# Ryannasr11/m2-tts

Hardware: AMD Instinct MI355X
Metric: audio samples/sec (22.05 kHz) + RTF, stage1_poc batch=32 @1/2/4/8 MI355X (higher is better)
Workload: dtype f32 (split 3xf16 MFMA, fp32 accumulate); 1 GPU; stage1_poc SimpleVocoder B=32 per GPU (configs[1]); stage=s1, per_gpu_batch=32, mel_frames=500, audio_samples_per_utt=32000, parallelism=weak-scaled replicas x1 (dp1, no collective in the data path)

## Files before the change

### m2-tts_amd/csrc/m2_common.h

```cpp
#pragma once

#include <hip/hip_runtime.h>
#include <stdint.h>
#include <string>

#include "../../include/m2tts_hip.h"

namespace m2 {

constexpr int kWave = 64;
constexpr float kLnEps = 1e-5f;
constexpr float kLeaky = 0.1f;
constexpr float kMaskFill = -1e9f;

enum Act : int { ACT_NONE = 0, ACT_LEAKY = 1, ACT_TANH = 2, ACT_RELU = 3, ACT_SOFTPLUS = 4 };

void set_error(const std::string& msg);

struct Switches {
    int dur_rb = 0;
    int dur_count = -1;
    int speculative = 1;
    bool tf_chain = true;
    bool tf_layer = true;
// ... 2 lines not shown
    int tfl_rb = 0;
    int tfl_first_rb = 0;
    int tfl_rb_masked = 0;
    int tfl_rb_unmasked = 0;
    int tfl_qs2 = -1;
    int att_qt = 0;
    bool att_f32 = false;
    bool voc_perlayer = false;
    bool voc_f32 = false;
    bool voc_tail_x3 = false;
    bool voc_mid_x3 = false;
    int voc_plan = -1;
    int f32_mt = 2;
    bool f32_pair = true;
    int x3_head_prio = 0;
    bool f32_comp = true;
    int midp_nch = 0;
    int tailp_nch = 0;
    bool tailp_seven = false;
    int tailp2_nch = 0;
    bool tailp2_seven = false;
    bool head_inconv = false;
    bool headmid = true;
    int s2_mid_alt = -1;
    int s2_head_tf = 0;
    int redo_grid = -1;
    bool redo_launch = false;
    bool dur_split = true;
    bool dur_pers = true;
};
const Switches& sw();
void reload_switches();

int32_t fail(int32_t code, const char* what);
int32_t hip_status(hipError_t e, const char* where);

#define M2_CHECK_ARG(cond, msg)                      \
    do {                                             \
        if (!(cond)) return ::m2::fail(M2_E_ARG, msg); \
    } while (0)
#define M2_CHECK_SHAPE(cond, msg)                      \
    do {                                               \
        if (!(cond)) return ::m2::fail(M2_E_SHAPE, msg); \
    } while (0)
#define M2_HIP(expr)                                                   \
    do {                                                               \
// ... 5 lines not shown
        hipError_t _e = hipGetLastError();                             \
        if (_e != hipSuccess) return ::m2::hip_status(_e, name);       \
    } while (0)

__device__ __forceinline__ float apply_act(float v, int act) {
    if (act == ACT_LEAKY) return v > 0.f ? v : v * kLeaky;
    if (act == ACT_TANH) return tanhf(v);
    if (act == ACT_RELU) return v > 0.f ? v : 0.f;
    if (act == ACT_SOFTPLUS) return v > 20.f ? v : log1pf(expf(v));
    return v;
}

template <int ACT>
__device__ __forceinline__ float act_t(float v) {
    if constexpr (ACT == ACT_LEAKY) return fmaxf(v, v * kLeaky);
    else if constexpr (ACT == ACT_TANH) return tanhf(v);
    else if constexpr (ACT == ACT_RELU) return v > 0.f ? v : 0.f;
    else return v;
}

__device__ __forceinline__ int dev_frames(const int32_t* p, int cap) {
    const int t = max(1, *p);
    return t <= cap ? t : 0;
}

inline int cdiv(int a, int b) { return (a + b - 1) / b; }
inline size_t align_up(size_t v, size_t a) { return (v + a - 1) / a * a; }

struct Carve {
    char* base;
    size_t cap;
    size_t off = 0;
    bool ok = true;
    Carve(void* p, size_t n) : base(static_cast<char*>(p)), cap(n) {}
    template <typename T>
    T* take(size_t count) {
        size_t o = align_up(off, 256);
        size_t n = count * sizeof(T);
        if (o + n > cap || base == nullptr) { ok = false; off = o + n; return nullptr; }
        off = o + n;
        return reinterpret_cast<T*>(base + o);
    }
};

struct Sizer {
    size_t off = 0;
// ... 43 lines not shown
```

### m2-tts_amd/csrc/m2_runtime.hip

```cpp
#include <immintrin.h>

#include <atomic>
#include <climits>
#include <cmath>
#include <cstdlib>
#include <cstring>
#include <mutex>
#include <new>
#include <string>
#include <vector>

#include "m2_common.h"
#include "m2_model.h"
#include "transformer_fused.h"
#include "transformer_layer.h"
#include "vocoder_fused.h"

namespace m2 {

namespace {
std::atomic<const Switches*> g_swp{nullptr};
std::mutex g_sw_mu;
int env_int(const char* name, int dflt) {
    const char* e = std::getenv(name);
// ... 32 lines not shown
        const int v = std::atoi(e);
        s.tfl_qs2 = (v == 2 || v == 3 || v == 4 || v == 12) ? v : 0;
    }
    s.att_qt = env_int("M2_ATT_QT", 0);
    if (const char* e = std::getenv("M2_ATT_F32")) s.att_f32 = *e && *e != '0';
    s.voc_perlayer = env_set("M2_VOCODER_PERLAYER");
    s.voc_f32 = env_set("M2_VOC_F32");
    s.voc_tail_x3 = env_set("M2_VOC_TAIL_X3");
    s.voc_mid_x3 = env_set("M2_VOC_MID_X3");
    s.voc_plan = env_int("M2_VOC_PLAN", -1);
    s.f32_mt = env_int("M2_F32_MT", 2);
    s.f32_pair = env_int("M2_F32_PAIR", 1) != 0;
    s.f32_comp = env_int("M2_F32_COMP", 1) != 0;
    s.x3_head_prio = env_int("M2_X3_HEAD_PRIO", 0);
    const int mn = env_int("M2_MIDP_NCH", 0);
    s.midp_nch = mn > 0 ? mn : 0;
    const int tn = env_int("M2_TAILP_NCH", 0);
    s.tailp_nch = tn > 0 ? tn : 0;
    s.tailp_seven = env_set("M2_TAILP_SEVEN");
    s.tailp2_nch = env_int("M2_TAILP2_NCH", 0);
    s.tailp2_seven = env_set("M2_TAILP2_SEVEN");
    s.head_inconv = env_set("M2_HEAD_INCONV");
    if (const char* e = std::getenv("M2_HEADMID"); e && (e[0] == '0' || e[0] == '1') && !e[1]) s.headmid = e[0] == '1';
    const int malt = env_int("M2_S2_MID_ALT", -1);
    s.s2_mid_alt = (malt == 0 || malt == 1) ? malt : -1;
    const int htf = env_int("M2_S2_HEAD_TF", env_set("M2_S2_HEAD_TF16") ? 16 : 0);
    s.s2_head_tf = (htf == 16 || htf == 19 || htf == 24 || htf == 27) ? htf : 0;
    s.redo_grid = env_int("M2_REDO_GRID", -1);
    s.redo_launch = env_set("M2_REDO_LAUNCH");
    s.dur_split = env_on("M2_DUR_SPLIT", true);
    s.dur_pers = env_on("M2_DUR_PERS", true);
    std::lock_guard<std::mutex> lk(g_sw_mu);
    const Switches* cur = g_swp.load(std::memory_order_relaxed);
    if (cur && std::memcmp(cur, &s, sizeof(Switches)) == 0) {
        std::free(raw);
        return;
    }
    g_swp.store(&s, std::memory_order_release);
}

int32_t launch_embed_pe(const int64_t*, const float*, const float*, int, int, int, int, float*, const int64_t*,
                        uint8_t*, hipStream_t);
int32_t launch_layer_norm(const float*, const float*, const float*, int, int, float*, hipStream_t);
int32_t launch_linear(const float*, const float*, const float*, const float*, const float*,
                      const float*, int, int, int, int, float*, hipStream_t);
int32_t launch_attention(const float*, const uint8_t*, int, int, int, int, float*, hipStream_t, bool force_f32 = false);
// ... 1259 lines not shown
```

### m2-tts_amd/csrc/vocoder_midp.h

```cpp
#pragma once
#include "m2_common.h"
#include "vocoder_fused.h"
#include "vocoder_pipe.h"

namespace m2 {
namespace mp {

using namespace pipe;

constexpr int RROWS = 64;
constexpr int RS0 = 288;
constexpr int RS1 = 544;

struct RingLay {
    static constexpr bool PLANES = false;
    static constexpr int R0_OFF = 0, R1_OFF = RROWS * RS0, R2_OFF = R1_OFF + RROWS * RS1;
    static constexpr int U_OFF = 0;
    static constexpr int LDS_BYTES = R2_OFF + RROWS * RS1;
};

constexpr int PROWS = 64, PRS = 288;

__device__ __forceinline__ unsigned r12_at(int row, int u) { return row * RS1 + 16 * (u ^ ((row >> 2) & 1)); }

template <int L, int S, class Lay = RingLay, int HB = 0, int NH = 2>
__device__ __forceinline__ void layer_role(unsigned char* lds, int qa, int L1, int nch, bool edge,
                                           const u32x4* __restrict__ W, const float* __restrict__ bias,
                                           unsigned char* __restrict__ u2row, int xown) {
    constexpr int NKB = mkb(L);
    constexpr bool PL = L == 0 && Lay::PLANES;
    constexpr int IN_OFF = L == 0 ? Lay::R0_OFF : (L == 1 ? Lay::R1_OFF : Lay::R2_OFF);
    constexpr int LO_IN = L == 0 ? 128 : 256;
    const int lane = threadIdx.x & 63, li = lane & 15, g = lane >> 4;
    u32x4 a[NH][NKB][2];
    float bv[NH][4];
#pragma unroll
    for (int hh = 0; hh < NH; ++hh) {
        const int h = HB + hh;
#pragma unroll
        for (int kb = 0; kb < NKB; ++kb) {
            const int u = munit0(L) + (2 * S + h) * NKB + kb;
            a[hh][kb][0] = W[u * 128 + lane];
            a[hh][kb][1] = W[u * 128 + 64 + lane];
        }
#pragma unroll
        for (int r = 0; r < 4; ++r) bv[hh][r] = bias[L * 128 + 32 * S + 16 * h + 4 * g + r];
    }
    unsigned radr[NKB][4], xadr[4], oadr[4];
#pragma unroll
    for (int j = 0; j < 4; ++j) {
#pragma unroll
        for (int kb = 0; kb < NKB; ++kb) {
            const MSlot sl = mslot(L, S, kb, g);
            if constexpr (PL) {
                const int e0 = li + sl.dq + 3, v = e0 & 3, row0 = (e0 >> 2) + (v >= 2 ? 1 : 0);
                radr[kb][j] = Lay::U_OFF + (v * PROWS + row0) * PRS + 16 * (sl.oct ^ (((row0 >> 2) + j) & 1));
            } else {
                const int row = (16 * j + li + sl.dq - 1) & (RROWS - 1);
                radr[kb][j] = IN_OFF + (L == 0 ? row * RS0 + sl.oct * 16 : r12_at(row, sl.oct));
            }
        }
        xadr[j] = Lay::R1_OFF + r12_at((16 * j + li - 2) & (RROWS - 1), 4 * S + g);
        oadr[j] = (L == 0 ? Lay::R1_OFF : Lay::R2_OFF) +
                  r12_at((16 * j + li) & (RROWS - 1), 4 * S + 16 * (g & 1) + (g >> 1));
    }
    u32x4 aid[NH];
// ... 43 lines not shown
#pragma unroll
            for (int r = 0; r < 4; ++r) v[r] = acc[hh][r];
            if constexpr (L < 2) {
                leaky4(v);
                if (straddle) {
                    const int x = x0 + li;
                    if (x < 0 || x >= L1) {
#pragma unroll
                        for (int r = 0; r < 4; ++r) v[r] = 0.f;
                    }
                }
            }
            unsigned h0, h1, l0, l1;
            split2u(v[0], v[1], h0, l0);
            split2u(v[2], v[3], h1, l1);
            const auto s0 = __builtin_amdgcn_permlane16_swap(h0, l0, false, false);
            const auto s1 = __builtin_amdgcn_permlane16_swap(h1, l1, false, false);
            const u32x4 val{s0[0], s1[0], s0[1], s1[1]};
            if constexpr (L < 2) {
                *reinterpret_cast<u32x4*>(lds + oadr[j] + 32 * h) = val;
            } else {
                const int x = x0 + li;
                if (k >= 0 && x >= 0 && x < xown)
                    *reinterpret_cast<u32x4*>(u2row + ((size_t)4 * x + S) * 128 + 32 * h + 64 * (g & 1) +
                                              16 * (g >> 1)) = val;
            }
        }
    };
    const int LAST = nch + 2;
    auto step = [&](int s, auto jc) {
        if (s <= LAST) {
            const int k = s - (L + 1);
            if (k >= -1 && k < nch) work(k, jc);
            step_barrier();
        }
    };
    constexpr int J0 = (-1 - (L + 1)) & 3;
#pragma unroll 1
    for (int s = -1; s <= LAST; s += 4) {
        step(s, ic<J0>{});
        step(s + 1, ic<(J0 + 1) & 3>{});
        step(s + 2, ic<(J0 + 2) & 3>{});
        step(s + 3, ic<(J0 + 3) & 3>{});
    }
}

}
}
// ... 1 lines not shown
```

### m2-tts_amd/csrc/vocoder_tailp.hip

```cpp
#include <algorithm>
#include <cstdlib>
#include <vector>

#include "m2_common.h"
#include "vocoder_fused.h"
#include "vocoder_pipe.h"

namespace m2 {
namespace tp {

using namespace pipe;

constexpr int kRingRows[7] = {64, 64, 64, 64, 64, 64, 48};
constexpr int kRingOff(int n) { return n == 0 ? 0 : kRingOff(n - 1) + kRingRows[n - 1] * 128; }
constexpr int kLoOff(int n) { return kRingRows[n] * 64; }
constexpr int kPeriod(int n) { return kRingRows[n] / 16; }
constexpr int kCorrSlot = kRingOff(6);
constexpr int ring_bytes(int nl) { return nl == 6 ? kCorrSlot + 16 : kRingOff(nl); }
constexpr int kFlagOff(int nl) { return ring_bytes(nl); }
constexpr int lds_bytes(int nl) { return ring_bytes(nl) + 16; }
constexpr int nwaves(int nl) { return nl + 1; }
static_assert(lds_bytes(6) * 3 <= 160 * 1024, "three workgroups per CU");
static_assert(lds_bytes(7) * 2 <= 160 * 1024, "two workgroups per CU");
#ifdef M2_STAMPS
constexpr int NWAVES = 8;
#endif

__device__ __forceinline__ unsigned ring_at(int n, int row, int oct) {
    return kRingOff(n) + row * 64 + 16 * (oct ^ ((row >> 1) & 3));
// ... 91 lines not shown
#pragma unroll
            for (int pr = 0; pr < 3; ++pr)
#pragma unroll
                for (int m = 0; m < NMB; ++m)
                    if (kb < nkbm(L, m)) {
                        const int f = frag(L, m, kb);
                        acc[m] = mfma_h(a[m][kb][pr == 2], pr == 1 ? bl[f] : bh[f], acc[m]);
                    }
        if constexpr (RES) {
#pragma unroll
            for (int m = 0; m < NMB; ++m) acc[m] = mfma_h(aid[m], xh, acc[m]);
#pragma unroll
            for (int m = 0; m < NMB; ++m) acc[m] = mfma_h(aid[m], xl, acc[m]);
        }
        const int x0 = sL + 16 * k;
        if constexpr (L == NL - 1) {
            const int x = x0 + li;
            if (g == 0 && k >= 0 && x >= 0 && x < L2) {
                float4 o;
                o.x = tanh_fast(acc[0][0]);
                o.y = tanh_fast(acc[0][1]);
                o.z = tanh_fast(acc[0][2]);
                o.w = tanh_fast(acc[0][3]);
                *reinterpret_cast<float4*>(arow + 4 * (size_t)x) = o;
                flag_nonfinite4(o.x, o.y, o.z, o.w, rflag, reinterpret_cast<int*>(lds + kFlagOff(NL)));
            }
        } else {
            auto epilogue = [&](auto zc) {
                constexpr bool ZERO = decltype(zc)::value;
                float v[NMB][4];
#pragma unroll
                for (int m = 0; m < NMB; ++m) {
#pragma unroll
                    for (int r = 0; r < 4; ++r) v[m][r] = acc[m][r];
                    if constexpr (ACT == ACT_LEAKY) leaky4(v[m]);
                }
                if constexpr (ZERO) {
                    const int x = x0 + li;
                    const bool out = x < 0 || x >= L2;
#pragma unroll
                    for (int m = 0; m < NMB; ++m)
#pragma unroll
                        for (int r = 0; r < 4; ++r) v[m][r] = out ? 0.f : v[m][r];
                    if constexpr (L == 4 && NL == 6) {
                        const float* cp = bias + kOutcCorr;
                        asm volatile("" : "+s"(cp));
                        const bool right = g >= 2;
// ... 73 lines not shown
#pragma unroll
        for (int f = 0; f < NF; ++f) {
            bh[f] = *reinterpret_cast<const u32x4*>(lds + radr(f, j));
            bl[f] = *reinterpret_cast<const u32x4*>(lds + radr(f, j) + (f < 2 ? kLoOff(5) : kLoOff(4)));
        }
        const int x0 = qa + 16 * k, x = x0 + li;
        f32x4 acc = f32x4{bv[0], bv[1], bv[2], bv[3]};
#pragma unroll
        for (int f = 0; f < NF; ++f)
#pragma unroll
            for (int pr = 0; pr < 3; ++pr) acc = mfma_h(a[f][pr == 2], pr == 1 ? bl[f] : bh[f], acc);
        float v[4] = {acc[0], acc[1], acc[2], acc[3]};
        if (edge && (x0 <= 0 || x0 + 16 >= L2)) {
            const f32x4 e = *reinterpret_cast<const f32x4*>(lds + kCorrSlot);
            if (x == 0) v[0] -= e[0] + e[1];
            if (x == L2 - 1) v[3] -= e[2] + e[3];
        }
        if (g == 0 && k >= 0 && x >= 0 && x < L2) {
            float4 o;
            o.x = tanh_fast(v[0]);
            o.y = tanh_fast(v[1]);
            o.z = tanh_fast(v[2]);
            o.w = tanh_fast(v[3]);
            *reinterpret_cast<float4*>(arow + 4 * (size_t)x) = o;
            flag_nonfinite4(o.x, o.y, o.z, o.w, rflag, reinterpret_cast<int*>(lds + kFlagOff(NL)));
        }
    };
    const int LAST = last_step(nch, NL);
    auto step = [&](int s, auto jc) {
        if (s <= LAST) {
            const int k = s - off_l(L);
            if (k >= 0 && k < nch) work(k, jc);
            step_barrier();
        }
    };
    constexpr int J0 = ((-1 - off_l(L)) % P + P) % P;
#pragma unroll 1
    for (int s = -1; s <= LAST; s += P) {
        step(s, ic<J0 % P>{});
        step(s + 1, ic<(J0 + 1) % P>{});
        step(s + 2, ic<(J0 + 2) % P>{});
        step(s + 3, ic<(J0 + 3) % P>{});
    }
}

template <int NL>
__device__ __forceinline__ void loader_role_dma(unsigned char* lds, int qa, int L2, int nch,
// ... 146 lines not shown
```

### m2-tts_amd/csrc/vocoder_x3.hip

```cpp
#include <cmath>
#include <cstdlib>
#include <cstring>
#include <type_traits>
#include <atomic>
#include <functional>

#include "m2_common.h"
#include "vocoder_fused.h"
#include "vocoder_launch.h"
#include "vocoder_midp.h"

namespace m2 {
namespace x3 {

typedef _Float16 h8 __attribute__((ext_vector_type(8)));
typedef _Float16 h4 __attribute__((ext_vector_type(4)));
typedef vx_u32x4 u32x4;
typedef float f32x4 __attribute__((ext_vector_type(4)));


__device__ __forceinline__ f32x4 mfma_h(u32x4 a, u32x4 b, f32x4 c) {
    return __builtin_amdgcn_mfma_f32_16x16x32_f16(__builtin_bit_cast(h8, a), __builtin_bit_cast(h8, b), c, 0, 0, 0);
}

// ... 470 lines not shown
    f32x4 acc[1][NT];
    f32x4 bv;
#pragma unroll
    for (int r = 0; r < 4; ++r) bv[r] = bias[ph * COUT + co0 + r];
#pragma unroll
    for (int n = 0; n < NT; ++n) acc[0][n] = bv;
    mma_x3<MP, 4, -1, RSM, NT, false, 1, NKB * 128, true>(wp, bp, nullptr, acc, *ap, wp_next);
    const int L = 4 * T, qe = ph < 2 ? 0 : T - 1;
#pragma unroll
    for (int n = 0; n < NT; ++n) {
        const int q = qs + 16 * n + li, t = 4 * q + ph;
        if (corr && qe >= qs + 16 * n && qe < qs + 16 * n + 16) {
            if (q == qe) {
                const f32x4 c = *reinterpret_cast<const f32x4*>(corr + 4 * (ph * COUT + co0));
#pragma unroll
                for (int r = 0; r < 4; ++r) acc[0][n][r] -= c[r];
            }
        }
        store_row<COUT, ACT_LEAKY, false, false>(acc[0][n], u + (pv * kPlane + 16 * n + li) * RSO, nullptr, co0,
                                                 t < 0 || t >= L, true, nullptr, t, plane_sw(li));
    }
}

template <int C, int RS, bool CONV2, bool INPL = false>
__device__ __forceinline__ void head_rb1_planar(const u32x4* __restrict__ Wp, const float* __restrict__ bias,
                                                const unsigned char* in, unsigned char* out,
                                                const unsigned char* x, int f0, int tf, int L, APipe* ap,
                                                const u32x4* wp_next, unsigned char* gout, int rot = 0) {
    constexpr int MB = C / 16, NKB = nkb_of<C, 3>(), NT = 4;
    static_assert(CONV2 || !INPL, "in place: conv2 only");
    const int item = __builtin_amdgcn_readfirstlane(threadIdx.x >> 6);
    const int p = item / MB, mb = item - p * MB;
    const int lane = threadIdx.x & 63, li = lane & 15, g = lane >> 4, co0 = mb * 16 + 4 * g;
    const int qo = CONV2 ? f0 : qs_h(p, f0);
    const unsigned char* tb[3];
#pragma unroll
    for (int d = 0; d < 3; ++d) {
        const int pd = p + d - 1, dq = pd < 0 ? -1 : (pd > 3 ? 1 : 0), pi = pd - 4 * dq;
        const int qsi = CONV2 ? qs_h(pi, f0) : qs_u(pi, f0);
        const int r = qo + dq - qsi + li;
        tb[d] = in + (pi * kPlane + r) * RS + 16 * (g ^ plane_sw(r));
    }
    const u32x4* wp = Wp + (size_t)mb * NKB * 128 + lane;
    f32x4 acc[1][NT];
    f32x4 bv;
#pragma unroll
    for (int r = 0; r < 4; ++r) bv[r] = bias[co0 + r];
#pragma unroll
    for (int n = 0; n < NT; ++n) acc[0][n] = bv;
    mma_x3<C, 3, 1, RS, NT, false, 1, NKB * 128, true, true>(wp, nullptr, nullptr, acc, *ap, wp_next, tb);
#pragma unroll
    for (int n = 0; n < NT; ++n) {
        const int q = qo + 16 * n + li, t = 4 * q + p + rot;
        if constexpr (INPL) {
            const int xr = q - qs_u(p, f0);
// ... 115 lines not shown
        const int _wg = blockIdx.y * gridDim.x + blockIdx.x;                                             \
        if ((threadIdx.x & 63) == 0 && _wg < 4096) g_x3_stamps[K][_wg][threadIdx.x >> 6][i] = _t;        \
    } while (0)
#define XSTAMP_RT(K, i)                                                                                  \
    do {                                                                                                 \
        __builtin_amdgcn_sched_barrier(0);                                                               \
        unsigned long long _t;                                                                           \
        asm volatile("s_memrealtime %0\n\ts_waitcnt lgkmcnt(0)" : "=s"(_t)::"memory");                  \
        __builtin_amdgcn_sched_barrier(0);                                                               \
        const int _wg = blockIdx.y * gridDim.x + blockIdx.x;                                             \
        if ((threadIdx.x & 63) == 0 && _wg < 4096) g_x3_stamps[K][_wg][threadIdx.x >> 6][i] = _t;        \
    } while (0)
#else
#define XSTAMP(K, i) \
    do {             \
    } while (0)
#define XSTAMP_RT(K, i) \
    do {                \
    } while (0)
#endif

template <class Cfg, bool TRANS, bool COMP = false>
__global__ __launch_bounds__(Cfg::HW * 64, Cfg::HMIN) void x3_head_kernel(const float* __restrict__ mel, int T,
                                                                            VocX w, unsigned char* __restrict__ U1) {
    if (w.rclear && blockIdx.x == 0 && blockIdx.y == 0 && threadIdx.x < 5) {
        if (threadIdx.x == 0) *reinterpret_cast<volatile int*>(w.rclear) = 0;
        else if (w.rqueue) reinterpret_cast<volatile unsigned*>(w.rqueue)[threadIdx.x - 1] = 0u;
    }
    if (w.head_prio == 1) {
        const int pr = __builtin_amdgcn_readfirstlane(threadIdx.x >> 6) >> 2;
        if (pr == 1) __builtin_amdgcn_s_setprio(1);
        else if (pr == 2) __builtin_amdgcn_s_setprio(2);
        else if (pr >= 3) __builtin_amdgcn_s_setprio(3);
    }
    constexpr int M = Cfg::M, MP = Cfg::MP, C = Cfg::C, TF = Cfg::TF;
    const int wx = blockIdx.x, wy = blockIdx.y;
    if (w.dT) {
        T = dev_frames(w.dT, T);
        if (wx * TF >= T) return;
    }
    using Pl = HeadPlan<MP, C, TF, head_planar<Cfg>()>;
    constexpr int C1 = Pl::C1;
    extern __shared__ __attribute__((aligned(16))) unsigned char lds[];
    const int b = wy, f0 = wx * TF;
    XW a0w{lds, f0 - 2};
    XW hw{lds, 4 * f0 - 1};
    XW melw{lds + Pl::RA, f0 - 3};
// ... 51 lines not shown
            ap[kb][0][1] = wp0[kb * 128 + 64];
        }
        static_assert(Pl::CAP_MEL * Pl::RS_M + 4 * 4 * C1 <= Pl::RA, "mel window + edge terms in region A");
        const XW melA{lds, f0 - 3};
        unsigned char* corr = lds + Pl::CAP_MEL * Pl::RS_M;
        const bool left = f0 == 0, right = T - 1 >= f0 - 1 && T - 1 < f0 + TF;
        float4 ev[4];
        float eb = 0.f;
        if (left || right) head_edge_load<MP, C1>(w.hce, ev, eb);
        gload_mel<TRANS, M, MP, Pl::RS_M, Pl::MEL_N, Cfg::HW * 64>(mel + (size_t)b * M * T, T, melA);
        XSTAMP(0, 1);
        __syncthreads();
        if (left || right) {
            head_edge_terms<MP, C1, Pl::RS_M>(ev, eb, melA, T, left, right, corr);
            __syncthreads();
        }
        XSTAMP(0, 2);
        XSTAMP(0, 3);
        XSTAMP(0, 4);
        unsigned char* up = lds + Pl::RA;
        unsigned char* hp = lds;
        head_convT1c_planar<MP, C1, Pl::RS_M, Pl::RS_1>(
            w.hc, w.hcb, (left || right) ? corr : nullptr, melA, up, f0, T, &ap,
            w.w1[0] + (size_t)(wv % MB1) * nkb_of<C1, 3>() * 128 + (threadIdx.x & 63));
        XSTAMP(0, 5);
        __syncthreads();
        XSTAMP(0, 6);
        head_rb1_planar<C1, Pl::RS_1, false>(w.w1[0], w.b1[0], up, hp, nullptr, f0, TF, 4 * T, &ap,
                                             w.w2[0] + (size_t)(wv % MB1) * nkb_of<C1, 3>() * 128 +
                                                 (threadIdx.x & 63),
                                             nullptr);
        XSTAMP(0, 7);
        __syncthreads();
        XSTAMP(0, 8);
        head_rb1_planar<C1, Pl::RS_1, true>(w.w2[0], w.b2[0], hp, nullptr, up, f0, TF, 4 * T, &ap, nullptr,
                                            U1 + (size_t)b * 4 * T * 4 * C1);
        XSTAMP(0, 9);
        XSTAMP_RT(0, 15);
        return;
    } else if constexpr (ONE) {
        const int wv = __builtin_amdgcn_readfirstlane(threadIdx.x >> 6);
        APipe ap;
        const u32x4* wp0 = I0::wp(w.wi, wv);
#pragma unroll
        for (int kb = 0; kb < 4; ++kb) {
            ap[kb][0][0] = wp0[kb * 128];
            ap[kb][0][1] = wp0[kb * 128 + 64];
        }
        gload_mel<TRANS, M, MP, Pl::RS_M, Pl::MEL_N, Cfg::HW * 64>(mel + (size_t)b * M * T, T, melw);
        XSTAMP(0, 1);
        __syncthreads();
        XSTAMP(0, 2);
        static_assert(PLANAR, "one item per wave: the phase-planar head");
        unsigned char* up = lds + Pl::RA;
        unsigned char* hp = lds;
        xconv3<MP, C, Cfg::NT_IN, ACT_NONE, false, Pl::RS_M, Pl::RS_C, Pl::A0_N, 1, NW>(
            w.wi, w.bi, melw, a0w, f0 - 2, T, &ap, w.wt[0] + (size_t)wv * nkb_of<C, 2>() * 128 + (threadIdx.x & 63));
        XSTAMP(0, 3);
        __syncthreads();
        XSTAMP(0, 4);
        constexpr int MB1 = C1 / 16;
        head_convT1_planar<C, C1, Pl::RS_C, Pl::RS_1>(w.wt[0], w.bt[0], a0w, up, f0, 4 * T, &ap,
                                                    w.w1[0] + (size_t)(wv % MB1) * nkb_of<C1, 3>() * 128 +
                                                        (threadIdx.x & 63));
        XSTAMP(0, 5);
        __syncthreads();
        XSTAMP(0, 6);
        head_rb1_planar<C1, Pl::RS_1, false>(w.w1[0], w.b1[0], up, hp, nullptr, f0, TF, 4 * T, &ap,
                                             w.w2[0] + (size_t)(wv % MB1) * nkb_of<C1, 3>() * 128 +
                                                 (threadIdx.x & 63),
                                             nullptr);
        XSTAMP(0, 7);
        __syncthreads();
        XSTAMP(0, 8);
        head_rb1_planar<C1, Pl::RS_1, true>(w.w2[0], w.b2[0], hp, nullptr, up, f0, TF, 4 * T, &ap, nullptr,
                                            U1 + (size_t)b * 4 * T * 4 * C1);
        XSTAMP(0, 9);
        XSTAMP_RT(0, 15);
        return;
    } else {
        gload_mel<TRANS, M, MP, Pl::RS_M, Pl::MEL_N, Cfg::HW * 64>(mel + (size_t)b * M * T, T, melw);
        XSTAMP(0, 1);
        __syncthreads();
        XSTAMP(0, 2);
        xconv3<MP, C, Cfg::NT_IN, ACT_NONE, false, Pl::RS_M, Pl::RS_C, Pl::A0_N>(w.wi, w.bi, melw, a0w, f0 - 2, T);
        XSTAMP(0, 3);
        __syncthreads();
        XSTAMP(0, 4);
        xconvT<C, C1, 4, Cfg::NT_T1, Pl::RS_C, Pl::RS_1, Pl::NQ>(w.wt[0], w.bt[0], a0w, uw, f0 - 1, 4 * T);
        XSTAMP(0, 5);
        __syncthreads();
        XSTAMP(0, 6);
        xconv3<C1, C1, Cfg::NT_R1, ACT_LEAKY, false, Pl::RS_1, Pl::RS_1, Pl::H_N>(w.w1[0], w.b1[0], uw, hw, 4 * f0 - 1,
                                                                                 4 * T);
        XSTAMP(0, 7);
        __syncthreads();
        XSTAMP(0, 8);
        xconv3<C1, C1, Cfg::NT_R1, ACT_NONE, true, Pl::RS_1, Pl::RS_1, Pl::O_N>(w.w2[0], w.b2[0], hw, uw, 4 * f0, 4 * T);
    }
    XSTAMP(0, 9);
    __syncthreads();
    XSTAMP(0, 10);
    gstore_rows<C1, Pl::RS_1, Pl::O_N, Cfg::HW * 64>(U1 + (size_t)b * 4 * T * 4 * C1, 4 * T, uw, 4 * f0);
    XSTAMP(0, 11);
}

struct HmPlan {
    using Pl = HeadPlan<CfgS1::MP, CfgS1::C, CfgS1::TF, true>;
    static constexpr int S_MAX = kHeadmidSMax;
    static_assert(Pl::LDS_BYTES == kHeadmidLds, "the plan's LDS bytes");
    struct Lay {
        static constexpr bool PLANES = true;
        static constexpr int R0_OFF = 0, R1_OFF = 0, R2_OFF = mp::RROWS * mp::RS1;
        static constexpr int U_OFF = Pl::RA;
    };
    static constexpr int NCH_MAX = (S_MAX + 15) / 16;
    static_assert(head_planar<CfgS1>() && CfgS1::HW == 16, "the phase-planar head of 16 waves");
    static_assert(Pl::RS_1 == mp::PRS && kPlane == mp::PROWS, "layer 0 of the mid reads the head's u planes");
    static_assert(Lay::R2_OFF + mp::RROWS * mp::RS1 <= Pl::RA, "rings R1 and R2 in region A");
    static_assert(Lay::U_OFF >= 4 * mp::PRS, "the warm-up chunk's rows stay inside LDS");
    static_assert(Lay::U_OFF + (3 * mp::PROWS + 4 * NCH_MAX + 2) * mp::PRS <= Pl::LDS_BYTES,
                  "the last chunk's rows stay inside LDS");
};

template <bool TRANS, int NCHC>
__global__ __launch_bounds__(CfgS1::HW * 64, CfgS1::HMIN) void headmid_kernel(const float* __restrict__ mel, int T,
                                                                               VocX w, unsigned char* __restrict__ U2,
                                                                               int S, int nch_arg) {
    if (w.rclear && blockIdx.x == 0 && blockIdx.y == 0 && threadIdx.x < 5) {
        if (threadIdx.x == 0) *reinterpret_cast<volatile int*>(w.rclear) = 0;
        else if (w.rqueue) reinterpret_cast<volatile unsigned*>(w.rqueue)[threadIdx.x - 1] = 0u;
    }
    const int wv = __builtin_amdgcn_readfirstlane(threadIdx.x >> 6);
    if (w.head_prio == 1) {
        const int pr = wv >> 2;
        if (pr == 1) __builtin_amdgcn_s_setprio(1);
        else if (pr == 2) __builtin_amdgcn_s_setprio(2);
        else if (pr >= 3) __builtin_amdgcn_s_setprio(3);
    }
    using Cfg = CfgS1;
    using Pl = HmPlan::Pl;
    using Lay = HmPlan::Lay;
    constexpr int M = Cfg::M, MP = Cfg::MP, TF = Cfg::TF, C1 = Pl::C1, MB1 = C1 / 16;
    extern __shared__ __attribute__((aligned(16))) unsigned char lds[];
    const int nch = NCHC ? NCHC : nch_arg;
    const int b = blockIdx.y, qa = blockIdx.x * S, L1 = 4 * T;
    const int o = qa - 1, f0 = o >> 2, rot = o & 3;
    APipe ap;
    {
        const int it0 = (((wv / MB1) + rot) & 3) * MB1 + wv % MB1;
        const u32x4* wp0 = w.hc + (size_t)it0 * nkb_of<MP, 4>() * 128 + (threadIdx.x & 63);
#pragma unroll
        for (int kb = 0; kb < 4; ++kb) {
            ap[kb][0][0] = wp0[kb * 128];
            ap[kb][0][1] = wp0[kb * 128 + 64];
        }
    }
    static_assert(Pl::CAP_MEL * Pl::RS_M + 4 * 4 * C1 <= Pl::RA, "mel window + edge terms in region A");
    const XW melA{lds, f0 - 3};
    unsigned char* corr = lds + Pl::CAP_MEL * Pl::RS_M;
    const bool left = f0 <= 1, right = T - 1 >= f0 - 1 && T - 1 <= f0 + 64;
    float4 ev[4];
    float eb = 0.f;
    if (left || right) head_edge_load<MP, C1>(w.hce, ev, eb);
    gload_mel<TRANS, M, MP, Pl::RS_M, Pl::MEL_N, Cfg::HW * 64>(mel + (size_t)b * M * T, T, melA);
    __syncthreads();
    if (left || right) {
        head_edge_terms<MP, C1, Pl::RS_M>(ev, eb, melA, T, left, right, corr);
        __syncthreads();
    }
    unsigned char* up = lds + Pl::RA;
    unsigned char* hp = lds;
    const u32x4* wr1 = w.w1[0] + (size_t)(wv % MB1) * nkb_of<C1, 3>() * 128 + (threadIdx.x & 63);
    const u32x4* wr2 = w.w2[0] + (size_t)(wv % MB1) * nkb_of<C1, 3>() * 128 + (threadIdx.x & 63);
    head_convT1c_planar<MP, C1, Pl::RS_M, Pl::RS_1>(w.hc, w.hcb, (left || right) ? corr : nullptr, melA, up, f0, T,
                                                    &ap, wr1, rot);
    __syncthreads();
    head_rb1_planar<C1, Pl::RS_1, false>(w.w1[0], w.b1[0], up, hp, nullptr, f0, TF, L1, &ap, wr2, nullptr, rot);
    __syncthreads();
    head_rb1_planar<C1, Pl::RS_1, true, true>(w.w2[0], w.b2[0], hp, nullptr, up, f0, TF, L1, &ap, nullptr, nullptr,
                                              rot);
    __syncthreads();
    const bool edge = qa < 16 || qa + 16 * nch + 16 > L1;
    const int xown = min(L1, qa + S);
    unsigned char* u2row = U2 + (size_t)b * 4 * L1 * 128;
    const u32x4* W = w.mp;
    const float* bias = w.mpb;
    const int layer = wv < 12 ? wv >> 2 : 3;
    if (layer == 2) __builtin_amdgcn_s_setprio(2);
    else if (layer == 1) __builtin_amdgcn_s_setprio(1);
    else __builtin_amdgcn_s_setprio(0);
    switch (wv) {
        case 0: mp::layer_role<0, 0, Lay>(lds, qa, L1, nch, edge, W, bias, u2row, xown); break;
        case 1: mp::layer_role<0, 1, Lay>(lds, qa, L1, nch, edge, W, bias, u2row, xown); break;
        case 2: mp::layer_role<0, 2, Lay>(lds, qa, L1, nch, edge, W, bias, u2row, xown); break;
        case 3: mp::layer_role<0, 3, Lay>(lds, qa, L1, nch, edge, W, bias, u2row, xown); break;
        case 4: mp::layer_role<1, 0, Lay>(lds, qa, L1, nch, edge, W, bias, u2row, xown); break;
        case 5: mp::layer_role<1, 1, Lay>(lds, qa, L1, nch, edge, W, bias, u2row, xown); break;
        case 6: mp::layer_role<1, 2, Lay>(lds, qa, L1, nch, edge, W, bias, u2row, xown); break;
        case 7: mp::layer_role<1, 3, Lay>(lds, qa, L1, nch, edge, W, bias, u2row, xown); break;
        case 8: mp::layer_role<2, 0, Lay>(lds, qa, L1, nch, edge, W, bias, u2row, xown); break;
        case 9: mp::layer_role<2, 1, Lay>(lds, qa, L1, nch, edge, W, bias, u2row, xown); break;
        case 10: mp::layer_role<2, 2, Lay>(lds, qa, L1, nch, edge, W, bias, u2row, xown); break;
        case 11: mp::layer_role<2, 3, Lay>(lds, qa, L1, nch, edge, W, bias, u2row, xown); break;
        default:
#pragma unroll 1
            for (int s = -1; s <= nch + 2; ++s) pipe::step_barrier();
            break;
    }
}

std::atomic<long> g_headmid_launches{0};

template <class Cfg>
__global__ __launch_bounds__(Cfg::MW * 64, Cfg::MMIN) void x3_mid_kernel(const unsigned char* __restrict__ U1,
                                                                           int L1, VocX w,
                                                                           unsigned char* __restrict__ U2) {
    constexpr int CI = Cfg::C / 2, W = Cfg::W2;
    using Pl = MidPlan<CI, W>;
    constexpr int CO = Pl::CO;
    extern __shared__ __attribute__((aligned(16))) unsigned char lds[];
    const int b = blockIdx.y, p0 = blockIdx.x * W;
    if (w.dT) {
        L1 = 4 * dev_frames(w.dT, L1 / 4);
        if (p0 >= L1) return;
    }
    const int L2 = 4 * L1;
// ... 137 lines not shown

struct Setup {
    hipError_t err;
    VocSlots slots;
};
const Setup& setup() {
    static const Setup s = [] {
        Setup r;
        r.err = set_rows_lds(reinterpret_cast<const KernelRow*>(&kRows), sizeof(Rows) / sizeof(KernelRow));
        auto head = [](VocHead h) { return row_slots(kRows.head[(int)h][1][0]); };
        r.slots = {head(VocHead::S2T16), head(VocHead::S2T19), head(VocHead::S2H24), head(VocHead::S2H27),
                   row_slots(kRows.mid[1]), row_slots(kRows.mid[2]), row_slots(kRows.tail[1]), row_slots(kRows.tail[2])};
        return r;
    }();
    return s;
}

int32_t run(const float* mel, int T, const VocLaunchPlan& p, const VocX& w, void* U1, void* U2, float* audio,
            hipStream_t st, const std::function<void(int, bool)>& mark) {
    if (setup().err != hipSuccess) return hip_status(setup().err, "x3 vocoder: hipFuncSetAttribute (one-time setup)");
    int32_t rc;
    int L1 = 4 * T, L2 = 16 * T;
    VocX wv = w;
    if (p.headmid) {
        void* args[] = {&mel, &T, &wv, &U2, const_cast<int*>(&p.hm_S), const_cast<int*>(&p.hm_nch)};
        if ((rc = launch_row(kRows.headmid[p.hm_nch == 16][p.trans], p.head_g, st, args, "headmid_kernel"))) return rc;
        g_headmid_launches.fetch_add(1, std::memory_order_relaxed);
    } else {
        mark(0, true);
        void* hargs[] = {&mel, &T, &wv, &U1};
        rc = launch_row(kRows.head[(int)p.head][p.comp][p.trans], p.head_g, st, hargs, "x3_head_kernel");
        mark(0, false);
        if (rc) return rc;
        mark(1, true);
        if (p.mid == VocMid::Midp) {
            rc = launch_vocoder_midp(U1, L1, p.mid_nch, p.mid_g, w.mp, w.mpb, U2, st, w.dT);
        } else {
            void* margs[] = {&U1, &L1, &wv, &U2};
            rc = launch_row(kRows.mid[p.mid == VocMid::X3Alt ? 2 : p.stage == 2], p.mid_g, st, margs,
                            "x3_mid_kernel");
        }
        if (rc) return rc;
        mark(1, false);
    }
    mark(2, true);
    if (p.tail == VocTail::Tailp2)
        rc = launch_vocoder_tailp2(U2, L2, p.tail_nl, p.tail_nch, p.tail_g, w.tp2, w.tp2b, audio, w.rflag, st, w.dT,
                                   VocRedo{w.redo_w, mel, p.trans});
    else if (p.tail == VocTail::Tailp)
        rc = launch_vocoder_tailp(U2, L2, p.tail_nl, p.tail_nch, p.tail_g, w.tp, w.tpb, audio, w.rflag, st, w.dT,
                                  VocRedo{w.redo_w, mel, p.trans});
    else {
        void* targs[] = {&U2, &L2, &wv, &audio};
// ... 150 lines not shown
```

Measured before the change: 16.01 billion audio samples/s.

## Add streaming stores, mb-major head work split, and role weight prefetch handover

Three changes to the vocoder kernels. Global 16-byte stores of U2 intermediates and final audio now go through buffer stores with a cache-policy bit (nontemporal/streaming by default) so write-once outputs do not pollute caches. The head rb1 stage can assign waves mb-major instead of position-major, changing which weight slices each wave loads. The last head conv also prefetches the first k-blocks of each mid-layer role's weights into the pipe registers and hands them over, hiding that load latency at the role start. Each is env- or macro-gated, and wrong cache bits or register pressure could hurt.

```diff
diff --git a/m2-tts_amd/csrc/m2_common.h b/m2-tts_amd/csrc/m2_common.h
--- a/m2-tts_amd/csrc/m2_common.h
+++ b/m2-tts_amd/csrc/m2_common.h
@@ -48,6 +48,7 @@
     bool tailp2_seven = false;
     bool head_inconv = false;
     bool headmid = true;
+    bool head_items = true;
     int s2_mid_alt = -1;
     int s2_head_tf = 0;
     int redo_grid = -1;
@@ -99,6 +100,19 @@
 __device__ __forceinline__ int dev_frames(const int32_t* p, int cap) {
     const int t = max(1, *p);
     return t <= cap ? t : 0;
+}
+
+template <int POLICY, class V>
+__device__ __forceinline__ void gstore16(void* base, size_t off, const V& v) {
+    static_assert(sizeof(V) == 16 && POLICY >= 0 && POLICY <= 2, "16-B vectors; policy 0, 1 or 2");
+    if constexpr (POLICY == 0) {
+        *reinterpret_cast<V*>(static_cast<unsigned char*>(base) + off) = v;
+    } else {
+        typedef unsigned gs_u32x4 __attribute__((ext_vector_type(4)));
+        const __amdgpu_buffer_rsrc_t rsrc = __builtin_amdgcn_make_buffer_rsrc(base, 0, -1, 0x00020000);
+        __builtin_amdgcn_raw_buffer_store_b128(__builtin_bit_cast(gs_u32x4, v), rsrc, (int)off, 0,
+                                               POLICY == 1 ? 16 : 2);
+    }
 }
 
 inline int cdiv(int a, int b) { return (a + b - 1) / b; }
diff --git a/m2-tts_amd/csrc/m2_runtime.hip b/m2-tts_amd/csrc/m2_runtime.hip
--- a/m2-tts_amd/csrc/m2_runtime.hip
+++ b/m2-tts_amd/csrc/m2_runtime.hip
@@ -78,6 +78,7 @@
     s.tailp2_seven = env_set("M2_TAILP2_SEVEN");
     s.head_inconv = env_set("M2_HEAD_INCONV");
     if (const char* e = std::getenv("M2_HEADMID"); e && (e[0] == '0' || e[0] == '1') && !e[1]) s.headmid = e[0] == '1';
+    s.head_items = env_int("M2_HEAD_ITEMS", 1) != 0;
     const int malt = env_int("M2_S2_MID_ALT", -1);
     s.s2_mid_alt = (malt == 0 || malt == 1) ? malt : -1;
     const int htf = env_int("M2_S2_HEAD_TF", env_set("M2_S2_HEAD_TF16") ? 16 : 0);
diff --git a/m2-tts_amd/csrc/vocoder_midp.h b/m2-tts_amd/csrc/vocoder_midp.h
--- a/m2-tts_amd/csrc/vocoder_midp.h
+++ b/m2-tts_amd/csrc/vocoder_midp.h
@@ -7,6 +7,10 @@
 namespace mp {
 
 using namespace pipe;
+
+#ifndef M2_U2_STORE
+#define M2_U2_STORE 1
+#endif
 
 constexpr int RROWS = 64;
 constexpr int RS0 = 288;
@@ -23,12 +27,19 @@
 
 __device__ __forceinline__ unsigned r12_at(int row, int u) { return row * RS1 + 16 * (u ^ ((row >> 2) & 1)); }
 
-template <int L, int S, class Lay = RingLay, int HB = 0, int NH = 2>
+constexpr int kPre = 4;
+__device__ __forceinline__ const u32x4* role_wp(const u32x4* __restrict__ W, int wv) {
+    const int l = wv >> 2, s = wv & 3;
+    return W + (size_t)(munit0(l) + 2 * s * mkb(l)) * 128 + (threadIdx.x & 63);
+}
+template <int L, int S, class Lay = RingLay, int HB = 0, int NH = 2, bool PRE = false>
 __device__ __forceinline__ void layer_role(unsigned char* lds, int qa, int L1, int nch, bool edge,
                                            const u32x4* __restrict__ W, const float* __restrict__ bias,
-                                           unsigned char* __restrict__ u2row, int xown) {
+                                           unsigned char* __restrict__ u2row, int xown,
+                                           const u32x4 (*pre)[1][2] = nullptr) {
     constexpr int NKB = mkb(L);
     constexpr bool PL = L == 0 && Lay::PLANES;
+    static_assert(NH * NKB >= kPre, "a role holds at least the handed-over k-blocks");
     constexpr int IN_OFF = L == 0 ? Lay::R0_OFF : (L == 1 ? Lay::R1_OFF : Lay::R2_OFF);
     constexpr int LO_IN = L == 0 ? 128 : 256;
     const int lane = threadIdx.x & 63, li = lane & 15, g = lane >> 4;
@@ -40,8 +51,13 @@
 #pragma unroll
         for (int kb = 0; kb < NKB; ++kb) {
             const int u = munit0(L) + (2 * S + h) * NKB + kb;
-            a[hh][kb][0] = W[u * 128 + lane];
-            a[hh][kb][1] = W[u * 128 + 64 + lane];
+            if (PRE && hh * NKB + kb < kPre) {
+                a[hh][kb][0] = pre[hh * NKB + kb][0][0];
+                a[hh][kb][1] = pre[hh * NKB + kb][0][1];
+            } else {
+                a[hh][kb][0] = W[u * 128 + lane];
+                a[hh][kb][1] = W[u * 128 + 64 + lane];
+            }
         }
 #pragma unroll
         for (int r = 0; r < 4; ++r) bv[hh][r] = bias[L * 128 + 32 * S + 16 * h + 4 * g + r];
@@ -131,8 +147,8 @@
             } else {
                 const int x = x0 + li;
                 if (k >= 0 && x >= 0 && x < xown)
-                    *reinterpret_cast<u32x4*>(u2row + ((size_t)4 * x + S) * 128 + 32 * h + 64 * (g & 1) +
-                                              16 * (g >> 1)) = val;
+                    gstore16<M2_U2_STORE>(u2row, ((size_t)4 * x + S) * 128 + 32 * h + 64 * (g & 1) + 16 * (g >> 1),
+                                          val);
             }
         }
     };
diff --git a/m2-tts_amd/csrc/vocoder_tailp.hip b/m2-tts_amd/csrc/vocoder_tailp.hip
--- a/m2-tts_amd/csrc/vocoder_tailp.hip
+++ b/m2-tts_amd/csrc/vocoder_tailp.hip
@@ -5,6 +5,10 @@
 #include "m2_common.h"
 #include "vocoder_fused.h"
 #include "vocoder_pipe.h"
+
+#ifndef M2_AUDIO_STORE
+#define M2_AUDIO_STORE 1
+#endif
 
 namespace m2 {
 namespace tp {
@@ -142,7 +146,7 @@
                 o.y = tanh_fast(acc[0][1]);
                 o.z = tanh_fast(acc[0][2]);
                 o.w = tanh_fast(acc[0][3]);
-                *reinterpret_cast<float4*>(arow + 4 * (size_t)x) = o;
+                gstore16<M2_AUDIO_STORE>(arow, 16 * (size_t)x, o);
                 flag_nonfinite4(o.x, o.y, o.z, o.w, rflag, reinterpret_cast<int*>(lds + kFlagOff(NL)));
             }
         } else {
@@ -262,7 +266,7 @@
             o.y = tanh_fast(v[1]);
             o.z = tanh_fast(v[2]);
             o.w = tanh_fast(v[3]);
-            *reinterpret_cast<float4*>(arow + 4 * (size_t)x) = o;
+            gstore16<M2_AUDIO_STORE>(arow, 16 * (size_t)x, o);
             flag_nonfinite4(o.x, o.y, o.z, o.w, rflag, reinterpret_cast<int*>(lds + kFlagOff(NL)));
         }
     };
diff --git a/m2-tts_amd/csrc/vocoder_x3.hip b/m2-tts_amd/csrc/vocoder_x3.hip
--- a/m2-tts_amd/csrc/vocoder_x3.hip
+++ b/m2-tts_amd/csrc/vocoder_x3.hip
@@ -516,15 +516,20 @@
     }
 }
 
+template <int MB>
+__device__ __forceinline__ int rb1_mb(int wv, bool mbmajor) {
+    return mbmajor ? wv / 4 : wv % MB;
+}
 template <int C, int RS, bool CONV2, bool INPL = false>
 __device__ __forceinline__ void head_rb1_planar(const u32x4* __restrict__ Wp, const float* __restrict__ bias,
                                                 const unsigned char* in, unsigned char* out,
                                                 const unsigned char* x, int f0, int tf, int L, APipe* ap,
-                                                const u32x4* wp_next, unsigned char* gout, int rot = 0) {
+                                                const u32x4* wp_next, unsigned char* gout, int rot = 0,
+                                                bool mbmajor = false) {
     constexpr int MB = C / 16, NKB = nkb_of<C, 3>(), NT = 4;
     static_assert(CONV2 || !INPL, "in place: conv2 only");
     const int item = __builtin_amdgcn_readfirstlane(threadIdx.x >> 6);
-    const int p = item / MB, mb = item - p * MB;
+    const int p = mbmajor ? item % 4 : item / MB, mb = rb1_mb<MB>(item, mbmajor);
     const int lane = threadIdx.x & 63, li = lane & 15, g = lane >> 4, co0 = mb * 16 + 4 * g;
     const int qo = CONV2 ? f0 : qs_h(p, f0);
     const unsigned char* tb[3];
@@ -686,7 +691,8 @@
 
 template <class Cfg, bool TRANS, bool COMP = false>
 __global__ __launch_bounds__(Cfg::HW * 64, Cfg::HMIN) void x3_head_kernel(const float* __restrict__ mel, int T,
-                                                                            VocX w, unsigned char* __restrict__ U1) {
+                                                                            VocX w, unsigned char* __restrict__ U1,
+                                                                            int items) {
     if (w.rclear && blockIdx.x == 0 && blockIdx.y == 0 && threadIdx.x < 5) {
         if (threadIdx.x == 0) *reinterpret_cast<volatile int*>(w.rclear) = 0;
         else if (w.rqueue) reinterpret_cast<volatile unsigned*>(w.rqueue)[threadIdx.x - 1] = 0u;
@@ -784,19 +790,19 @@
         unsigned char* hp = lds;
         head_convT1c_planar<MP, C1, Pl::RS_M, Pl::RS_1>(
             w.hc, w.hcb, (left || right) ? corr : nullptr, melA, up, f0, T, &ap,
-            w.w1[0] + (size_t)(wv % MB1) * nkb_of<C1, 3>() * 128 + (threadIdx.x & 63));
+            w.w1[0] + (size_t)rb1_mb<MB1>(wv, items) * nkb_of<C1, 3>() * 128 + (threadIdx.x & 63));
         XSTAMP(0, 5);
         __syncthreads();
         XSTAMP(0, 6);
         head_rb1_planar<C1, Pl::RS_1, false>(w.w1[0], w.b1[0], up, hp, nullptr, f0, TF, 4 * T, &ap,
-                                             w.w2[0] + (size_t)(wv % MB1) * nkb_of<C1, 3>() * 128 +
+                                             w.w2[0] + (size_t)rb1_mb<MB1>(wv, items) * nkb_of<C1, 3>() * 128 +
                                                  (threadIdx.x & 63),
-                                             nullptr);
+                                             nullptr, 0, items);
         XSTAMP(0, 7);
         __syncthreads();
         XSTAMP(0, 8);
         head_rb1_planar<C1, Pl::RS_1, true>(w.w2[0], w.b2[0], hp, nullptr, up, f0, TF, 4 * T, &ap, nullptr,
-                                            U1 + (size_t)b * 4 * T * 4 * C1);
+                                            U1 + (size_t)b * 4 * T * 4 * C1, 0, items);
         XSTAMP(0, 9);
         XSTAMP_RT(0, 15);
         return;
@@ -823,20 +829,20 @@
         XSTAMP(0, 4);
         constexpr int MB1 = C1 / 16;
         head_convT1_planar<C, C1, Pl::RS_C, Pl::RS_1>(w.wt[0], w.bt[0], a0w, up, f0, 4 * T, &ap,
-                                                    w.w1[0] + (size_t)(wv % MB1) * nkb_of<C1, 3>() * 128 +
+                                                    w.w1[0] + (size_t)rb1_mb<MB1>(wv, items) * nkb_of<C1, 3>() * 128 +
                                                         (threadIdx.x & 63));
         XSTAMP(0, 5);
         __syncthreads();
         XSTAMP(0, 6);
         head_rb1_planar<C1, Pl::RS_1, false>(w.w1[0], w.b1[0], up, hp, nullptr, f0, TF, 4 * T, &ap,
-                                             w.w2[0] + (size_t)(wv % MB1) * nkb_of<C1, 3>() * 128 +
+                                             w.w2[0] + (size_t)rb1_mb<MB1>(wv, items) * nkb_of<C1, 3>() * 128 +
                                                  (threadIdx.x & 63),
-                                             nullptr);
+                                             nullptr, 0, items);
         XSTAMP(0, 7);
         __syncthreads();
         XSTAMP(0, 8);
         head_rb1_planar<C1, Pl::RS_1, true>(w.w2[0], w.b2[0], hp, nullptr, up, f0, TF, 4 * T, &ap, nullptr,
-                                            U1 + (size_t)b * 4 * T * 4 * C1);
+                                            U1 + (size_t)b * 4 * T * 4 * C1, 0, items);
         XSTAMP(0, 9);
         XSTAMP_RT(0, 15);
         return;
@@ -867,6 +873,9 @@
     XSTAMP(0, 11);
 }
 
+#ifndef M2_ROLE_PREFETCH
+#define M2_ROLE_PREFETCH 1
+#endif
 struct HmPlan {
     using Pl = HeadPlan<CfgS1::MP, CfgS1::C, CfgS1::TF, true>;
     static constexpr int S_MAX = kHeadmidSMax;
@@ -888,7 +897,7 @@
 template <bool TRANS, int NCHC>
 __global__ __launch_bounds__(CfgS1::HW * 64, CfgS1::HMIN) void headmid_kernel(const float* __restrict__ mel, int T,
                                                                                VocX w, unsigned char* __restrict__ U2,
-                                                                               int S, int nch_arg) {
+                                                                               int S, int nch_arg, int items) {
     if (w.rclear && blockIdx.x == 0 && blockIdx.y == 0 && threadIdx.x < 5) {
         if (threadIdx.x == 0) *reinterpret_cast<volatile int*>(w.rclear) = 0;
         else if (w.rqueue) reinterpret_cast<volatile unsigned*>(w.rqueue)[threadIdx.x - 1] = 0u;
@@ -933,15 +942,18 @@
     }
     unsigned char* up = lds + Pl::RA;
     unsigned char* hp = lds;
-    const u32x4* wr1 = w.w1[0] + (size_t)(wv % MB1) * nkb_of<C1, 3>() * 128 + (threadIdx.x & 63);
-    const u32x4* wr2 = w.w2[0] + (size_t)(wv % MB1) * nkb_of<C1, 3>() * 128 + (threadIdx.x & 63);
+    const u32x4* wr1 = w.w1[0] + (size_t)rb1_mb<MB1>(wv, items) * nkb_of<C1, 3>() * 128 + (threadIdx.x & 63);
+    const u32x4* wr2 = w.w2[0] + (size_t)rb1_mb<MB1>(wv, items) * nkb_of<C1, 3>() * 128 + (threadIdx.x & 63);
     head_convT1c_planar<MP, C1, Pl::RS_M, Pl::RS_1>(w.hc, w.hcb, (left || right) ? corr : nullptr, melA, up, f0, T,
                                                     &ap, wr1, rot);
     __syncthreads();
-    head_rb1_planar<C1, Pl::RS_1, false>(w.w1[0], w.b1[0], up, hp, nullptr, f0, TF, L1, &ap, wr2, nullptr, rot);
-    __syncthreads();
-    head_rb1_planar<C1, Pl::RS_1, true, true>(w.w2[0], w.b2[0], hp, nullptr, up, f0, TF, L1, &ap, nullptr, nullptr,
-                                              rot);
+    head_rb1_planar<C1, Pl::RS_1, false>(w.w1[0], w.b1[0], up, hp, nullptr, f0, TF, L1, &ap, wr2, nullptr, rot,
+                                         items);
+    __syncthreads();
+    constexpr bool PREF = M2_ROLE_PREFETCH != 0;
+    static_assert(sizeof(APipe) == mp::kPre * 2 * sizeof(u32x4), "the hand-over holds the roles' first k-blocks");
+    head_rb1_planar<C1, Pl::RS_1, true, true>(w.w2[0], w.b2[0], hp, nullptr, up, f0, TF, L1, &ap,
+                                              PREF && wv < 12 ? mp::role_wp(w.mp, wv) : nullptr, nullptr, rot, items);
     __syncthreads();
     const bool edge = qa < 16 || qa + 16 * nch + 16 > L1;
     const int xown = min(L1, qa + S);
@@ -953,18 +965,18 @@
     else if (layer == 1) __builtin_amdgcn_s_setprio(1);
     else __builtin_amdgcn_s_setprio(0);
     switch (wv) {
-        case 0: mp::layer_role<0, 0, Lay>(lds, qa, L1, nch, edge, W, bias, u2row, xown); break;
-        case 1: mp::layer_role<0, 1, Lay>(lds, qa, L1, nch, edge, W, bias, u2row, xown); break;
-        case 2: mp::layer_role<0, 2, Lay>(lds, qa, L1, nch, edge, W, bias, u2row, xown); break;
-        case 3: mp::layer_role<0, 3, Lay>(lds, qa, L1, nch, edge, W, bias, u2row, xown); break;
-        case 4: mp::layer_role<1, 0, Lay>(lds, qa, L1, nch, edge, W, bias, u2row, xown); break;
-        case 5: mp::layer_role<1, 1, Lay>(lds, qa, L1, nch, edge, W, bias, u2row, xown); break;
-        case 6: mp::layer_role<1, 2, Lay>(lds, qa, L1, nch, edge, W, bias, u2row, xown); break;
-        case 7: mp::layer_role<1, 3, Lay>(lds, qa, L1, nch, edge, W, bias, u2row, xown); break;
-        case 8: mp::layer_role<2, 0, Lay>(lds, qa, L1, nch, edge, W, bias, u2row, xown); break;
-        case 9: mp::layer_role<2, 1, Lay>(lds, qa, L1, nch, edge, W, bias, u2row, xown); break;
-        case 10: mp::layer_role<2, 2, Lay>(lds, qa, L1, nch, edge, W, bias, u2row, xown); break;
-        case 11: mp::layer_role<2, 3, Lay>(lds, qa, L1, nch, edge, W, bias, u2row, xown); break;
+        case 0: mp::layer_role<0, 0, Lay, 0, 2, PREF>(lds, qa, L1, nch, edge, W, bias, u2row, xown, ap); break;
+        case 1: mp::layer_role<0, 1, Lay, 0, 2, PREF>(lds, qa, L1, nch, edge, W, bias, u2row, xown, ap); break;
+        case 2: mp::layer_role<0, 2, Lay, 0, 2, PREF>(lds, qa, L1, nch, edge, W, bias, u2row, xown, ap); break;
+        case 3: mp::layer_role<0, 3, Lay, 0, 2, PREF>(lds, qa, L1, nch, edge, W, bias, u2row, xown, ap); break;
+        case 4: mp::layer_role<1, 0, Lay, 0, 2, PREF>(lds, qa, L1, nch, edge, W, bias, u2row, xown, ap); break;
+        case 5: mp::layer_role<1, 1, Lay, 0, 2, PREF>(lds, qa, L1, nch, edge, W, bias, u2row, xown, ap); break;
+        case 6: mp::layer_role<1, 2, Lay, 0, 2, PREF>(lds, qa, L1, nch, edge, W, bias, u2row, xown, ap); break;
+        case 7: mp::layer_role<1, 3, Lay, 0, 2, PREF>(lds, qa, L1, nch, edge, W, bias, u2row, xown, ap); break;
+        case 8: mp::layer_role<2, 0, Lay, 0, 2, PREF>(lds, qa, L1, nch, edge, W, bias, u2row, xown, ap); break;
+        case 9: mp::layer_role<2, 1, Lay, 0, 2, PREF>(lds, qa, L1, nch, edge, W, bias, u2row, xown, ap); break;
+        case 10: mp::layer_role<2, 2, Lay, 0, 2, PREF>(lds, qa, L1, nch, edge, W, bias, u2row, xown, ap); break;
+        case 11: mp::layer_role<2, 3, Lay, 0, 2, PREF>(lds, qa, L1, nch, edge, W, bias, u2row, xown, ap); break;
         default:
 #pragma unroll 1
             for (int s = -1; s <= nch + 2; ++s) pipe::step_barrier();
@@ -1148,13 +1160,14 @@
     int32_t rc;
     int L1 = 4 * T, L2 = 16 * T;
     VocX wv = w;
+    int items = sw().head_items;
     if (p.headmid) {
-        void* args[] = {&mel, &T, &wv, &U2, const_cast<int*>(&p.hm_S), const_cast<int*>(&p.hm_nch)};
+        void* args[] = {&mel, &T, &wv, &U2, const_cast<int*>(&p.hm_S), const_cast<int*>(&p.hm_nch), &items};
         if ((rc = launch_row(kRows.headmid[p.hm_nch == 16][p.trans], p.head_g, st, args, "headmid_kernel"))) return rc;
         g_headmid_launches.fetch_add(1, std::memory_order_relaxed);
     } else {
         mark(0, true);
-        void* hargs[] = {&mel, &T, &wv, &U1};
+        void* hargs[] = {&mel, &T, &wv, &U1, &items};
         rc = launch_row(kRows.head[(int)p.head][p.comp][p.trans], p.head_g, st, hargs, "x3_head_kernel");
         mark(0, false);
         if (rc) return rc;
```

Result: faster. 17.42 billion audio samples/s, median of 6 (+8.8%).
